# joshspeagle/frankenz

Measured on AMD Instinct MI355X. Metric: object-template likelihood evals/sec (fused fit_predict -> PDFs), higher is better.
Workload: dtype f64 throughout (chi2, ln-likes, every weight, ln-evidence, PDFs; an fp32 estimate of the weight only CLASSIFIES which pairs can matter to an fp64 sum, DESIGN.md 3.1)

## Files before the change

### frankenz_amd/csrc/fz_hist.h

```cpp
#pragma once
#include <type_traits>
#include "fz_kernels.h"
#include "fz_nolist.h"

namespace fz {

#define FZ_HEXP_K 256
#ifndef FZ_HIST_MP
#define FZ_HIST_MP 1
#endif
#ifndef FZ_HIST_TILE384
#define FZ_HIST_TILE384 1
#endif
#ifndef FZ_HIST_REFRESH_TILE
#define FZ_HIST_REFRESH_TILE 1
#endif
#ifndef FZ_HIST_STAGE_LATE
#define FZ_HIST_STAGE_LATE 1
#endif
#ifndef FZ_HIST_SETTLE2
#define FZ_HIST_SETTLE2 0
#endif
#ifndef FZ_HIST_SEG_NW0
#define FZ_HIST_SEG_NW0 16
#endif
#ifndef FZ_HIST_SEG_PFMAX
#define FZ_HIST_SEG_PFMAX 12
#endif
#ifndef FZ_HIST_REFRESH
#define FZ_HIST_REFRESH 32
#endif
#ifndef FZ_HIST_LEAN
#define FZ_HIST_LEAN 1
#endif
#ifndef FZ_HIST_AHEAD
#define FZ_HIST_AHEAD 1
#endif
#ifndef FZ_HIST_WAIT_EARLY
#define FZ_HIST_WAIT_EARLY 0
#endif
#ifndef FZ_HIST_SEAM
#define FZ_HIST_SEAM 1
#endif
#ifndef FZ_HIST_PRIO
#define FZ_HIST_PRIO 1
#endif
constexpr int hist_prio_level(int policy, int pos) {
    return policy == 1 ? (pos < 2 ? 3 : (pos < 4 ? 2 : (pos < 5 ? 1 : 0)))
         : policy == 2 ? (pos < 3 ? 1 : 0)
         : policy == 3 ? (pos < 2 ? 1 : 0)
         : 0;
}
#ifndef FZ_HIST_PRIO_FORMS
#define FZ_HIST_PRIO_FORMS (2 | 4 | 8 | 16)
#endif
constexpr int hist_prio_step(int pos, int ns) { return ns < 2 ? 0 : (3 * (ns - 1 - pos) + ns - 2) / (ns - 1); }
__device__ __forceinline__ void hist_setprio(int p) {
    switch (p) {
        case 0: __builtin_amdgcn_s_setprio(0); break;
        case 1: __builtin_amdgcn_s_setprio(1); break;
        case 2: __builtin_amdgcn_s_setprio(2); break;
        default: __builtin_amdgcn_s_setprio(3); break;
    }
}
#ifdef FZ_HIST_WSTATS
static __device__ unsigned long long fz_hwstats[16 * 12];
#define FZ_HIST_WSTATS_ON 1
inline void hist_wstats_print(hipStream_t stream, int nb, long long n, long long M, long long blocks, int nw) {
    unsigned long long h[16 * 12], z[16 * 12] = {0};
    (void)hipStreamSynchronize(stream);
    (void)hipMemcpyFromSymbol(h, HIP_SYMBOL(fz_hwstats), sizeof h);
    (void)hipMemcpyToSymbol(HIP_SYMBOL(fz_hwstats), z, sizeof z);
    fprintf(stderr, "HWSTATS k_hist<%d bands>: n %lld M %lld, %lld blocks x %d waves\n", nb, n, M, blocks, nw);
    for (int r = 0; r < nw / 4; ++r) {
        double s[5] = {0, 0, 0, 0, 0};
        char simd[128]; int q = 0;
        for (int w = 4 * r; w < 4 * r + 4; ++w) {
            const unsigned long long* e = h + w * 12;
            for (int k = 0; k < 5; ++k) s[k] += (double)e[k];
            q += snprintf(simd + q, sizeof simd - q, " w%d:%llu/%llu/%llu/%llu", w, e[8], e[9], e[10], e[11]);
        }
        const double life = s[4] > 0 ? s[4] : 1.0;
        fprintf(stderr, "HWSTATS rank %d (waves %d-%d): life %.4g cycles per wave | tile barrier %.2f %% | round barriers %.2f %% | finish %.2f %% | "
                        "prologue %.2f %% | per wave, tile barrier %%:", r, 4 * r, 4 * r + 3, s[4] / (4.0 * (double)(h[4 * r * 12 + 5] ? h[4 * r * 12 + 5] : 1)),
                100 * s[0] / life, 100 * s[1] / life, 100 * s[2] / life, 100 * s[3] / life);
        for (int w = 4 * r; w < 4 * r + 4; ++w) fprintf(stderr, " %.2f", 100.0 * (double)h[w * 12] / (double)(h[w * 12 + 4] ? h[w * 12 + 4] : 1));
        fprintf(stderr, " | launches on SIMD 0/1/2/3:%s\n", simd);
    }
}
#else
#define FZ_HIST_WSTATS_ON 0
#endif
template <bool L>
__device__ __forceinline__ double fma3(double a, double b, double c) {
    if constexpr (L) { double d; asm("v_fma_f64 %0, %1, %2, %3" : "=v"(d) : "v"(a), "v"(b), "v"(c)); return d; }
    else return fma(a, b, c);
}
template <bool L>
__device__ __forceinline__ double fma3_sb(double a, double b, double c) {
    if constexpr (L) { double d; asm("v_fma_f64 %0, %1, %2, %3" : "=v"(d) : "v"(a), "s"(b), "v"(c)); return d; }
    else return fma(a, b, c);
}
template <bool L>
__device__ __forceinline__ double fma3_mhalf(double a, double c) {
    if constexpr (L) { double d; asm("v_fma_f64 %0, %1, -0.5, %2" : "=v"(d) : "v"(a), "v"(c)); return d; }
    else return fma(a, -0.5, c);
}
template <bool L>
__device__ __forceinline__ int exp_insert(int hi, int n) {
    if constexpr (L) { int r; asm("v_lshl_add_u32 %0, %1, 12, %2" : "=v"(r) : "v"(n & ~(FZ_HEXP_K - 1)), "v"(hi)); return r; }
    else return hi + ((n >> 8) << 20);
}
struct ExpK {
    double c1 = 369.3299304675746;
    double c2 = -0.0027076061740622863;
    double c6 = 1.0 / 6.0;
};
template <bool NEGONLY = false, bool L = false>
__device__ __forceinline__ double exp_small_tab(double x, const double* __restrict__ tab, const ExpK& ek = ExpK()) {
    const double MAGIC = 6755399441055744.0;
    x = NEGONLY ? vmax_raw(x, -700.0) : vmin_raw(vmax_raw(x, -700.0), 700.0);
    const double d = fma(x, ek.c1, MAGIC);
    const double r = fma(d - MAGIC, ek.c2, x);
    const int n = __double2loint(d);
    const double t = tab[n & (FZ_HEXP_K - 1)];
    double p = fma3_sb<L>(r, 1.0 / 120.0, 1.0 / 24.0);
    p = fma3<L>(p, r, ek.c6);
    p = fma(p, r, 0.5);
    p = fma(p, r, 1.0);
    p = fma(p, r, 1.0);
    const double v = t * p;
    static_assert(FZ_HEXP_K == 256, "the exponent insert shifts n by log2 of the table's length");
    return __hiloint2double(exp_insert<L>(__double2hiint(v), n), __double2loint(v));
}

__device__ __forceinline__ double sqrt_nr(double r) {
    const double y = __builtin_amdgcn_rsq(vmax_raw(r, 1e-300));
    const double hy = 0.5 * y;
    double s = r * y;
    s = fma(fma(-s, s, r), hy, s);
    s = fma(fma(-s, s, r), hy, s);
    return s;
}
constexpr double hist_ln(double k) {
    return k == 1.0 ? 0.0 : k == 2.0 ? 0.6931471805599453 : k == 3.0 ? 1.0986122886681098 : k == 4.0 ? 1.3862943611198906
         : k == 5.0 ? 1.6094379124341003 : k == 6.0 ? 1.791759469228055 : k == 7.0 ? 1.9459101090932196 : 2.0794415416798357;
}
template <int WP, bool SMALL = false, bool L = false>
__device__ __forceinline__ double hist_exactw(double c2, const FastTabs& tb, const ExpK& ek = ExpK()) {
    constexpr double K = (double)WP;
    const double r = c2 * (1.0 / K);
    double pw = 1.0;
    if constexpr ((WP >> 1) <= 3) {
        if constexpr ((WP >> 1) >= 1) pw = r;
        if constexpr ((WP >> 1) >= 2) pw = pw * r;
        if constexpr ((WP >> 1) >= 3) pw = pw * r;
    } else {
        double base = r;
#pragma unroll
        for (int e = WP >> 1; e > 0; e >>= 1) { if (e & 1) pw = pw * base; base = base * base; }
    }
    if constexpr (SMALL && (WP >> 1) <= 3) {
        double q = 1.0;
        if constexpr ((WP >> 1) >= 1) q = c2;
        if constexpr ((WP >> 1) >= 2) q = q * c2;
        if constexpr ((WP >> 1) >= 3) q = q * c2;
        if constexpr (WP & 1) {
            const double y = __builtin_amdgcn_rsq(c2), hy = 0.5 * y;
            double sq = c2 * y;
            sq = fma(fma(-sq, sq, c2), hy, sq);
            sq = fma(fma(-sq, sq, c2), hy, sq);
            q = (WP >> 1) ? q * sq : sq;
        }
        constexpr double EK = 0.5 * K - 0.5 * K * hist_ln(K);
        return q * exp_small_tab<true, L>(fma3_mhalf<L>(c2, EK), tb.expt, ek);
    }
    if constexpr (!SMALL && (WP >> 1) <= 3) {
        double q = 1.0;
        if constexpr ((WP >> 1) >= 1) q = c2;
        if constexpr ((WP >> 1) >= 2) q = q * c2;
        if constexpr ((WP >> 1) >= 3) q = q * c2;
        if constexpr (WP & 1) q = (WP >> 1) ? q * sqrt_nr(c2) : sqrt_nr(c2);
        constexpr double EK = 0.5 * K - 0.5 * K * hist_ln(K);
        return q * exp_neg(fma(c2, -0.5, EK), tb);
    }
    if constexpr (WP & 1) pw = pw * sqrt_nr(r);
    const double w = pw * (SMALL ? exp_small_tab(fma(c2, -0.5, 0.5 * K), tb.expt) : exp_clamped(fma(c2, -0.5, 0.5 * K), tb));
    if constexpr ((WP >> 1) > 3) return (c2 < K + 1400.0) ? w : 0.0;
    else return w;
}

template <bool SMALL = false>
__device__ __forceinline__ double hist_exactw_rt(double c2, int wp, const FastTabs& tb) {
    const double K = (double)wp;
    if (wp == 0) return SMALL ? exp_small_tab(-0.5 * c2, tb.expt) : exp_clamped(-0.5 * c2, tb);
    const double r = c2 * rcp_nr<2>(K);
    double pw = 1.0, base = r;
    for (int e = wp >> 1; e > 0; e >>= 1) { if (e & 1) pw = pw * base; base = base * base; }
    if (wp & 1) pw = pw * sqrt_nr(r);
    const double w = pw * (SMALL ? exp_small_tab(fma(c2, -0.5, 0.5 * K), tb.expt) : exp_clamped(fma(c2, -0.5, 0.5 * K), tb));
    return (c2 < K + 1400.0) ? w : 0.0;
}

template <bool SMALL = false>
__device__ __forceinline__ double hist_exactw_rt8(double c2, int wp, double K, double rK, const FastTabs& tb) {
    if (wp == 0) return SMALL ? exp_small_tab<true>(-0.5 * c2, tb.expt) : exp_clamped(-0.5 * c2, tb);
    const double r = c2 * rK, r2 = r * r;
    const int h = wp >> 1;
    double pw = ((h & 1) ? r : 1.0) * ((h & 2) ? r2 : 1.0);
    if (wp & 1) pw = pw * sqrt_nr(r);
    return pw * (SMALL ? exp_small_tab<true>(fma(c2, -0.5, 0.5 * K), tb.expt) : exp_clamped(fma(c2, -0.5, 0.5 * K), tb));
}

template <class SRC>
constexpr int hist_tile() {
    if (FZ_HIST_SETTLE2 && SRC::NB <= 8 && SRC::RW <= 6 && SRC::LMODE == 1) return 128;
    if (FZ_HIST_TILE384 && SRC::NB <= 8 && SRC::RW <= 6) return 384;
    if (SRC::NB <= 8) return (SRC::RW <= 10 && !(SRC::LMODE == 2 && SRC::RW > 6)) ? 256 : 128;
    return SRC::RW <= 18 ? 256 : (SRC::RW <= 34 ? 128 : 64);
}
template <class SRC>
constexpr bool hist_prefetch() {
    if (SRC::NB <= 8) return SRC::NB + SRC::NVAL <= 18;
    return 2 * SRC::NB + 2 * SRC::RW <= 96;
}

__device__ __forceinline__ float wave_maxf_dpp(float v) {
    int x = __float_as_int(v);
    auto mx = [](int a, int b) { float r; asm("v_max_f32 %0, %1, %2" : "=v"(r) : "v"(__int_as_float(a)), "v"(__int_as_float(b))); return __float_as_int(r); };
    x = mx(x, __builtin_amdgcn_update_dpp(x, x, 0xB1, 0xf, 0xf, false));
    x = mx(x, __builtin_amdgcn_update_dpp(x, x, 0x4E, 0xf, 0xf, false));
    x = mx(x, __builtin_amdgcn_update_dpp(x, x, 0x141, 0xf, 0xf, false));
    x = mx(x, __builtin_amdgcn_update_dpp(x, x, 0x140, 0xf, 0xf, false));
    const float a = __int_as_float(__builtin_amdgcn_readlane(x, 0)), b = __int_as_float(__builtin_amdgcn_readlane(x, 16));
    const float c = __int_as_float(__builtin_amdgcn_readlane(x, 32)), d = __int_as_float(__builtin_amdgcn_readlane(x, 48));
    return fmaxf(fmaxf(a, b), fmaxf(c, d));
}

__device__ __forceinline__ double wave_max_pos_hi(double v) {
    int x = __double2hiint(v);
    auto mx = [](int a, int b) { return a > b ? a : b; };
    x = mx(x, __builtin_amdgcn_update_dpp(x, x, 0xB1, 0xf, 0xf, false));
    x = mx(x, __builtin_amdgcn_update_dpp(x, x, 0x4E, 0xf, 0xf, false));
    x = mx(x, __builtin_amdgcn_update_dpp(x, x, 0x141, 0xf, 0xf, false));
    x = mx(x, __builtin_amdgcn_update_dpp(x, x, 0x140, 0xf, 0xf, false));
    const int a = __builtin_amdgcn_readlane(x, 0), b = __builtin_amdgcn_readlane(x, 16), c = __builtin_amdgcn_readlane(x, 32), d = __builtin_amdgcn_readlane(x, 48);
    return __hiloint2double(mx(mx(a, b), mx(c, d)), 0);
}

#ifndef FZ_HIST_CHI2_2OP
#define FZ_HIST_CHI2_2OP 1
#endif
#ifndef FZ_HIST_C2ZERO
#define FZ_HIST_C2ZERO 1e-16
#endif

template <int TW>
struct HistState {
    double S[TW];
    double Sc[TW];
    double wmx[TW];
    float tmax[TW];
    float tthr[TW];
    double wamb[TW];
    int pend[TW];
    int namb[TW];
    int tick, next;
};

template <class SRC>
struct HistArgs {
    SRC src;
    KdeView kv;
    int64_t N;
    double* lmap; double* levid; double* pdfs;
    const int* omap; int* redo; const int* order;
    int normalize;
};
template <class SRC, int TW, int NW, bool EXACT, bool OBJK = (SRC::NB > 8), bool SEG = false>
__global__ __launch_bounds__(NW * 64) void k_hist(HistArgs<SRC> a_, const KdeView* __restrict__ kvp, int acc_stride, int M,
                                                   double wt_thresh, Cand* __restrict__ amb, int64_t cap) {
    constexpr bool LEAN = (FZ_HIST_LEAN == 1) && !SEG;
    constexpr bool AHD = (FZ_HIST_AHEAD == 1) && LEAN && !EXACT && !(FZ_HIST_SETTLE2 == 1) && !OBJK && SRC::RW <= 6;
    constexpr bool WE = (FZ_HIST_WAIT_EARLY == 1) && AHD;
    constexpr bool SEAM = (FZ_HIST_SEAM == 1) && AHD && hist_prefetch<SRC>() && (FZ_HIST_STAGE_LATE == 1);
    auto hq = [&]() -> const HistArgs<SRC>& {
        if constexpr (!LEAN) return a_;
        auto p = __builtin_amdgcn_kernarg_segment_ptr();
        asm volatile("" : "+s"(p));
        return *(const HistArgs<SRC>*)p;
    };
    const int64_t N = a_.N;
    constexpr int TILE = hist_tile<SRC>(), RW = SRC::RW, TDR = RW * TILE, TD = TDR + TILE / 2, NT = NW * 64, OD = SRC::OBJ_DOUBLES;
    constexpr int WP = SRC::WPOW, BT = SRC::NB;
    constexpr int PRIO = (SEAM && TILE == 384 && (BT == 5 || (FZ_HIST_PRIO_FORMS & 16))) ? FZ_HIST_PRIO : 0;
    constexpr int PFORM = SEG ? 8 : (OBJK ? 2 : (EXACT ? 4 : 1));
    constexpr bool PWORSE = (SEG && !EXACT && SRC::LMODE == 0 && BT == 4) || (OBJK && !SEG && !EXACT && BT == 8);
    constexpr bool PRIOF = (FZ_HIST_PRIO > 0) && !SEAM && BT <= 8 && (FZ_HIST_PRIO_FORMS & PFORM) != 0 && !PWORSE;
    constexpr bool WST = (FZ_HIST_WSTATS_ON == 1) && SEAM;
    [[maybe_unused]] unsigned long long wst_a = 0, wst_b = 0, wst_c = 0, wst_d = 0;
    auto wclk = [&]() -> unsigned long long { if constexpr (WST) return __builtin_readcyclecounter(); else return 0ull; };
    [[maybe_unused]] const unsigned long long wst_life = wclk();
    static_assert(!OBJK || TW == 1, "per-object band counts: one object per wave");
    static_assert(!SEG || (OBJK && SRC::NB <= 8), "segments: run-time band counts, 4-8 bands");
    constexpr double SEG_VBIG = BT <= 5 ? 0x1p192 : (BT == 6 ? 0x1p160 : (BT == 7 ? 0x1p137 : 0x1p120));
    constexpr int KOFF = SRC::LMODE == 2 ? 3 : 2;
    constexpr bool KRT = OBJK;
    int wpr = WP;
    double K = (double)WP;
    bool kok = true;
    double lgq = a_.src.lp.lg_full;
    constexpr int NOBJ = NW * TW;
    constexpr bool S2 = (FZ_HIST_SETTLE2 == 1) && !EXACT && SRC::NB <= 8 && SRC::RW <= 6 && SRC::LMODE == 1;
    constexpr int CAP = S2 ? 192 : 128, DTHR = CAP - 64;
    using tag_t = uint16_t;
    static_assert(WP >= 1 && WP <= 30, "chi2^(1/2) ... chi2^15");
    __shared__ __attribute__((aligned(16))) double tileA[TD];
    __shared__ __attribute__((aligned(16))) double tileB[TD];
    __shared__ __attribute__((aligned(16))) double s_c2[EXACT ? 2 : NOBJ * CAP];
    __shared__ tag_t s_tag[EXACT ? 2 : NOBJ * CAP];
    __shared__ __attribute__((aligned(16))) double s_tabs[EXACT ? FZ_TABS_DOUBLES : FZ_HEXP_K];
    __shared__ __attribute__((aligned(16))) double s_objs[EXACT ? NOBJ * OD : 2];
    __shared__ __attribute__((aligned(16))) double s_obj0[SEG ? NOBJ * OD : 2];
    static_assert(EXACT || TW * OD <= TW * CAP, "an object row must fit its candidate buffer");
    extern __shared__ double s_rows[];
    const int tid = threadIdx.x, lane = tid & 63;
    const int wave = __builtin_amdgcn_readfirstlane(tid >> 6);
    const int64_t nwaves = (int64_t)gridDim.x * NW, gw = (int64_t)blockIdx.x * NW + wave;
    const int64_t ngroups = (N + TW - 1) / TW, nrounds = (ngroups + nwaves - 1) / nwaves;
    const int ntiles = (M + TILE - 1) / TILE;
    SRC src = a_.src;
    src.tb = global_tabs();
    const FastTabs tb = src.tb;
    FastTabs tbx;
    if constexpr (EXACT) tbx = stage_tabs(s_tabs, tid, NT);
    else {
        for (int k = tid; k < FZ_HEXP_K; k += NT) s_tabs[k] = FZ_EXP_TAB[k * (FZ_EXP_K / FZ_HEXP_K)];
        tbx.logt = nullptr; tbx.expt = s_tabs;
    }
    const KdeView kv = [&]() { if constexpr (SEG) return *kvp; else return a_.kv; }();
    const int32_t* posw = SEG ? kv.mc_tag : kv.pos;
    const int w0 = SEG ? 0 : kv.w0;
    double* objs = EXACT ? s_objs + wave * (TW * OD) : s_c2 + wave * (TW * CAP);
    double* obj0 = s_obj0 + (SEG ? wave * (TW * OD) : 0);
    double* rows = s_rows + (size_t)wave * TW * acc_stride;
    double* rc2 = s_c2 + (EXACT ? 0 : wave * (TW * CAP));
    tag_t* rtag = s_tag + (EXACT ? 0 : wave * (TW * CAP));
    Cand* ambw = amb + (size_t)gw * TW * cap;
    auto t_consts = [](double Kd, float& hk23, float& T0c, float& tmarg) {
        const double hk = 0.5 * Kd;
        hk23 = (float)(hk / 8388608.0);
        T0c = (float)((Kd > 0.0 ? -hk * log2(Kd) : 0.0) + Kd * 0.7213475204444817 + hk * (-127.0 + 0.043));
        tmarg = (float)(0.5 + 0.045 * hk);
    };
    float hk23, T0c, tmarg;
    t_consts(K, hk23, T0c, tmarg);
    float tzero = K > 0.0 ? -INFINITY : T0c;
    const float lthr2 = (wt_thresh > 0.0) ? (float)log2(wt_thresh) : -INFINITY;
    int mbits = 0;
    while (((int64_t)1 << mbits) < (int64_t)M) ++mbits;
    const float ldrop0 = fminf(lthr2, -(float)(55 + mbits));
    const double thr_def = wt_thresh * (1.0 + 1e-3);
    auto lnl_c2 = [&](double c2) {
        if constexpr (KRT) return (wpr == 0) ? fma(-0.5, c2, -lgq) : chi2_logpdf<true>(0.5 * K, c2, lgq, tb);
        else return src.lnl_of_chi2(c2);
    };
    double rK = 1.0;
    ExpK ek;
    if constexpr (LEAN) asm volatile("" : "+s"(ek.c1), "+s"(ek.c2), "+v"(ek.c6));
    auto exactw_tab = [&](double c2, const FastTabs& t, auto small) {
        if constexpr (SEG) {
            if constexpr (SRC::LMODE == 2) { if (wpr == WP) return hist_exactw<WP, decltype(small)::value>(c2, t); }
            return hist_exactw_rt8<decltype(small)::value>(c2, wpr, K, rK, t);
        }
        else if constexpr (KRT) return hist_exactw_rt<decltype(small)::value>(c2, wpr, t);
        else return hist_exactw<WP, decltype(small)::value, LEAN>(c2, t, ek);
    };
    double lref = uniform_d(lnl_c2(K));
    auto obj_of = [&](const HistArgs<SRC>& h, int64_t s) -> int64_t {
        if constexpr (!EXACT && !SEG) {
            if (h.order) { const int64_t q = (int64_t)h.order[s]; s = q < 0 ? 0 : (q < h.N ? q : h.N - 1); }
        }
        return h.omap ? (int64_t)h.omap[s] : s;
    };

    for (int64_t rnd = 0; rnd < nrounds; ++rnd) {
        const int64_t g = gw + rnd * nwaves;
        const bool work = g < ngroups;
        [[maybe_unused]] const unsigned long long wst_r0 = wclk();
        const int64_t i0 = work ? g * TW : 0;
        const HistArgs<SRC>& hp = hq();
        [[maybe_unused]] const SRC& srcp = hp.src;
#pragma unroll
        for (int o = 0; o < TW; ++o) {
            const int64_t os = i0 + o < hp.N ? i0 + o : hp.N - 1;
            srcp.park_obj(obj_of(hp, os), objs + o * OD, lane);
        }
        for (int k = lane; k < TW * acc_stride; k += 64) rows[k] = 0.0;
        uint32_t obits = 0; double oslv = 0.0, fk = 1.0; int segcur = -1, ndcur = 0;
        bool segbad = false;
        int nbadm = 0;
        auto seg_lnl = [&](double c2, int nd) {
            const bool dp = src.lp.dim_prior != 0;
            const int wp = dp ? nd - KOFF : 0;
            const double lg = dp ? src.lp.lgtab[nd] : 0.5 * ((double)nd * FZ_LN2PI + oslv);
            const double xl = (wp == 0) ? 0.0 : (0.5 * (double)wp) * log_pos_t<true>(c2, tb);
            return fma(-0.5, c2, xl) - lg;
        };
        if constexpr (SEG) {
            const int64_t os = i0 < hp.N ? i0 : hp.N - 1;
            const int64_t oi = obj_of(hp, os);
            src.park_obj(oi, obj0, lane);
            if constexpr ((SRC::LMODE == 1 || SRC::LMODE == 2) && FZ_HIST_CHI2_2OP && !(SRC::LMODE == 2 && SRC::SAFE)) {
                if (lane < BT) { const double sv = sqrt(obj0[BT + lane]); obj0[BT + lane] = sv; obj0[lane] = obj0[lane] * sv; }
            }
            obits = (uint32_t)__builtin_amdgcn_readfirstlane((int)src.ov.bits[oi]);
            oslv = uniform_d(src.ov.slv[oi]);
            const bool dp = src.lp.dim_prior != 0;
            double lr = -INFINITY; bool bad = false;
            for (int sg = lane; sg < kv.seg_n; sg += 64) {
                const int nd = __popc(obits & kv.seg_mask[sg]);
                const int wp = dp ? nd - KOFF : 0;
                bad |= wp < -1;
                nbadm += (wp == -1) ? kv.seg_start[sg + 1] - kv.seg_start[sg] : 0;
                const double lg = dp ? src.lp.lgtab[nd] : 0.5 * ((double)nd * FZ_LN2PI + oslv);
                const double hw = 0.5 * (double)wp;
                if (wp >= 0) lr = fmax(lr, wp > 0 ? fma(hw, log_pos((double)wp, tb), -hw) - lg : -lg);
            }
            nbadm = __builtin_amdgcn_readfirstlane((int)wave_sum((double)nbadm));
            kok = __ballot(bad) == 0ull && nbadm <= (M >> 3);
            lref = uniform_d(wave_max(lr));
            float h_, t_; t_consts((double)BT, h_, t_, tmarg);
            tmarg = uniform_f(tmarg);
        }
        if constexpr (OBJK && !SEG) {
            const int64_t os = i0 < hp.N ? i0 : hp.N - 1;
            const int64_t oi = obj_of(hp, os);
            const int nb = __builtin_amdgcn_readfirstlane(__popc(srcp.ov.bits[oi]));
            wpr = nb - (SRC::LMODE == 2 ? 3 : 2);
            kok = wpr >= 0;
            if (!kok) wpr = 1;
            const bool dp = src.lp.dim_prior != 0;
            if (!dp) { wpr = 0; kok = true; }
            K = uniform_d((double)wpr);
            t_consts(K, hk23, T0c, tmarg);
            hk23 = uniform_f(hk23); T0c = uniform_f(T0c); tmarg = uniform_f(tmarg);
            tzero = wpr > 0 ? -INFINITY : T0c;
            lgq = uniform_d(dp ? srcp.lp.lgtab[nb] : 0.5 * ((double)nb * FZ_LN2PI + srcp.ov.slv[oi]));
            lref = uniform_d(lnl_c2(K));
        }
        int tid0 = tid;
        if constexpr (SEAM) asm volatile("" : "+v"(tid0));
        nl_stage_tile<SRC, TILE, NT, true>(src, posw, 0, tileA, tid0, wave);
        if constexpr (WST) {
            const unsigned long long t1 = wclk();
// ... 333 lines not shown
                    if constexpr (SLOW) { const int lim = flush ? 1 : DTHR; while (hs.pend[o] >= lim) drain(o, std::true_type{}, lane); }
                    else { while (hs.pend[o] >= DTHR) drain(o, std::false_type{}, lane); }
#endif
                        }
                    }
                }
        };
        auto tile_barrier = [&]() {
#if !defined(FZ_DIAG_NOBARRIER)
            if constexpr (WST) {
                const unsigned long long t0 = wclk();
                __syncthreads();
                wst_a += wclk() - t0;
            } else
            __syncthreads();
#endif
        };
        [[maybe_unused]] typename SRC::MR mseam[MP];
        [[maybe_unused]] int tagseam[MP];
        auto run_tile = [&](const double* cur, double* nxt, int t, auto tailc, auto slowc) {
            constexpr bool TAIL = decltype(tailc)::value;
            constexpr bool pure = !decltype(slowc)::value;
            constexpr bool LATE = FZ_HIST_STAGE_LATE && pure && hist_prefetch<SRC>() && !(SEG && SRC::NB + SRC::NVAL > FZ_HIST_SEG_PFMAX);
            if (!LATE || !work) { if (t + 1 < ntiles) nl_stage_tile<SRC, TILE, NT, true>(src, posw, t + 1, nxt, tid, wave); }
            if (work) {
                const int32_t* tags = reinterpret_cast<const int32_t*>(cur + TDR);
                static_assert((TILE / 64) % MP == 0, "groups per trip must divide the tile");
                constexpr bool PF = hist_prefetch<SRC>() && !(SEG && SRC::NB + SRC::NVAL > FZ_HIST_SEG_PFMAX);
                if constexpr (pure) {
                    typename SRC::MR mn[PF ? MP : 1];
                    int tagn[MP];
                    if constexpr (SEAM) {
#pragma unroll
                        for (int q = 0; q < MP; ++q) { mn[q] = mseam[q]; tagn[q] = tagseam[q]; }
                    } else if constexpr (PF) {
#pragma unroll
                        for (int q = 0; q < MP; ++q) {
                            src.template load_model_lds<TILE>(cur, q * 64 + lane, mn[q]);
                            tagn[q] = tags[q * 64 + lane];
                        }
                    }
                    if constexpr (LATE) { if (t + 1 < ntiles) nl_stage_tile<SRC, TILE, NT, true>(src, posw, t + 1, nxt, tid, wave); }
#pragma unroll
                    for (int st = 0; st < TILE / 64; st += MP) {
                        typename SRC::MR m[MP];
                        int ptag[MP];
#pragma unroll
                        for (int q = 0; q < MP; ++q) {
                            if constexpr (PF) { m[q] = mn[q]; ptag[q] = tagn[q]; }
                            else { src.template load_model_lds<TILE>(cur, (st + q) * 64 + lane, m[q]); ptag[q] = tags[(st + q) * 64 + lane]; }
                            asm volatile("" : "+v"(ptag[q]));
                        }
                        if (PF && st + MP < TILE / 64) {
#pragma unroll
                            for (int q = 0; q < MP; ++q) {
                                src.template load_model_lds<TILE>(cur, (st + MP + q) * 64 + lane, mn[q]);
                                tagn[q] = tags[(st + MP + q) * 64 + lane];
                            }
                        }
                        if constexpr (SEAM) {
                            if (st + MP >= TILE / 64) {
                                tile_barrier();
                                if constexpr (!TAIL) {
                                    const int32_t* tagx = reinterpret_cast<const int32_t*>(nxt + TDR);
#pragma unroll
                                    for (int q = 0; q < MP; ++q) {
                                        src.template load_model_lds<TILE>(nxt, q * 64 + lane, mseam[q]);
                                        tagseam[q] = tagx[q * 64 + lane];
                                    }
                                }
                            }
                        }
                        if constexpr (PRIO >= 1 && PRIO <= 3) hist_setprio(hist_prio_level(PRIO, st + MP >= TILE / 64 ? 0 : st + 1));
                        if constexpr (PRIO == 5) { if (st == 0) hist_setprio(((wave >> 2) + t) & 3); }
                        if constexpr (PRIOF) hist_setprio(hist_prio_step(st / MP, TILE / 64 / MP));
                        if constexpr (AHD && PF) __builtin_amdgcn_sched_barrier(0);
                        step_body(m, ptag, st, t, tailc, std::false_type{}, false);
                    }
                } else {
                    {
#pragma unroll 1
                        for (int st = -1; st < TILE / 64; ++st) {
                            typename SRC::MR m[MP];
                            int ptag[MP];
                            const int stc = st < 0 ? 0 : st;
                            src.template load_model_lds<TILE>(cur, stc * 64 + lane, m[0]);
                            ptag[0] = st < 0 ? (int)0x80000000 : tags[stc * 64 + lane];
                            const int nxt = st + 1 < TILE / 64 ? (tags[(st + 1) * 64] >> 16) & 0x3fff : segcur;
                            if (st >= 0) {
                                const int sw = (__builtin_amdgcn_readfirstlane(ptag[0]) >> 16) & 0x7fff;
                                if ((sw & 0x3fff) != segcur) {
                                    if (mcw && segcur >= 0) {
                                        const int rko = kv.seg_rank[segcur];
                                        if (kv.seg_rank[sw & 0x3fff] != rko) { const HistArgs<SRC>& hc = hq(); class_flush(rko, rows, hc.pdfs + obj_of(hc, i0) * kv.G); }
                                    }
                                    seg_switch(sw);
                                }
                            }
                            const bool flush = __builtin_amdgcn_readfirstlane(nxt) != segcur;
                            step_body(m, ptag, stc, t, tailc, std::true_type{}, flush);
                        }
                    }
                }
                if constexpr (FZ_HIST_REFRESH_TILE && !EXACT) {
                    if (++hs.tick == hs.next) { hs.next = hs.tick < 3 ? hs.tick + 1 : hs.tick + 5; refresh_bars(); }
                }
            }
            if constexpr (SEAM && pure) { if (!work) tile_barrier(); }
            else tile_barrier();
        };
        if constexpr (SEAM) {
            if (work) {
                const int32_t* tag0 = reinterpret_cast<const int32_t*>(tileA + TDR);
#pragma unroll
                for (int q = 0; q < MP; ++q) {
                    src.template load_model_lds<TILE>(tileA, q * 64 + lane, mseam[q]);
                    tagseam[q] = tag0[q * 64 + lane];
                }
            }
        }
        if constexpr (PRIO == 4) { if (work) hist_setprio(wave >> 2); }
        if constexpr (!SEG) {
            for (int t = 0; t < ntiles; t += 2) {
                if (t + 1 < ntiles) run_tile(tileA, tileB, t, std::false_type{}, std::false_type{}); else run_tile(tileA, tileB, t, std::true_type{}, std::false_type{});
                if (t + 1 < ntiles) {
                    if (t + 2 < ntiles) run_tile(tileB, tileA, t + 1, std::false_type{}, std::false_type{}); else run_tile(tileB, tileA, t + 1, std::true_type{}, std::false_type{});
                }
            }
        } else {
            auto tile_pure = [&](const double* cur) -> bool {
                if (!work) return true;
                const int wv = (reinterpret_cast<const int32_t*>(cur + TDR)[(lane % (TILE / 64)) * 64] >> 16) & 0x7fff;
                return __ballot(wv != segcur) == 0ull && !segbad;
            };
            int t = 0;
            while (t < ntiles) {
                if (!(t & 1)) {
                    while (t < ntiles) {
                        if (!tile_pure(tileA)) break;
                        run_tile(tileA, tileB, t, std::false_type{}, std::false_type{}); ++t;
                        if (t >= ntiles || !tile_pure(tileB)) break;
                        run_tile(tileB, tileA, t, std::false_type{}, std::false_type{}); ++t;
                    }
                    if (t >= ntiles) break;
                }
                if (t & 1) run_tile(tileB, tileA, t, std::false_type{}, std::true_type{});
                else run_tile(tileA, tileB, t, std::false_type{}, std::true_type{});
                ++t;
            }
        }

        if constexpr (PRIO > 0 || PRIOF) __builtin_amdgcn_s_setprio(0);
        [[maybe_unused]] const unsigned long long wst_f0 = wclk();
        if (work) {
#pragma unroll 1
            for (int o = 0; o < TW; ++o) {
                const HistArgs<SRC>& hf = hq();
                const KdeView& kvf = SEG ? kv : hf.kv;
                if (i0 + o >= hf.N) break;
                const int64_t i = obj_of(hf, i0 + o);
                double* const pdfs = hf.pdfs;
                auto lnl_fin = [&](double c2) {
                    if constexpr (KRT || !LEAN) return lnl_c2(c2);
                    else return chi2_logpdf<true>(0.5 * WP, c2, hf.src.lp.lg_full, tb);
                };
                double lrf = lref;
                if constexpr (!KRT && LEAN) lrf = uniform_d(lnl_fin(K));
                double* row = rows + o * acc_stride;
                double wbest_run = 0.0;
                int lanef = lane;
                if constexpr (SEAM) asm volatile("" : "+v"(lanef));
                if constexpr (!EXACT) {
                    while (hs.pend[o] > 0) drain(o, std::integral_constant<bool, SEG>{}, lanef);
                } else {
                    wbest_run = wave_max(hs.Sc[o]);
                }
                if constexpr (!EXACT) wbest_run = wave_max(hs.wmx[o]);
                const double lbest = (wbest_run > 0.0) ? uniform_d(lrf + log_pos(wbest_run, tb)) : -INFINITY;
                const double stot = wave_sum(EXACT ? hs.S[o] : hs.Sc[o]);
                const double le = lrf + log_pos(stot, tb);
                const float tm = EXACT ? 0.f : wave_maxf(hs.tmax[o]);
                const bool ok = (le - le == 0.0) && (lbest > -INFINITY) && (EXACT ? (wbest_run > 1e-24) : (tm >= -400.f)) && hs.namb[o] >= 0 && kok;
                if constexpr (SEG) { if (mcw && segcur >= 0) class_flush(kv.seg_rank[segcur], row, pdfs + i * kv.G); }
                const int na = __builtin_amdgcn_readfirstlane(hs.namb[o]);
                if (na > 0) {
                    __builtin_amdgcn_fence(__ATOMIC_RELEASE, "workgroup");
                    __builtin_amdgcn_fence(__ATOMIC_ACQUIRE, "agent");
                    const double thr = wt_thresh * exp_neg(lbest - le, tb);
                    const Cand* cb = ambw + (size_t)o * cap;
                    for (int c0 = 0; c0 < na; c0 += 64) {
                        const int k = c0 + lane;
                        const bool in1 = k < na;
                        const Cand e1 = cb[in1 ? k : 0];
                        double l1, w1;
                        if constexpr (SEG) {
                            l1 = in1 ? seg_lnl(e1.lnl, e1.pad & 0xff) : -INFINITY;
                            w1 = exp_neg(l1 - lref, tb);
                        } else {
                            l1 = in1 ? lnl_fin(e1.lnl) : -INFINITY;
                            w1 = exactw_tab(e1.lnl, tb, std::false_type{});
                        }
                        const bool s1 = in1 && (exp_neg(l1 - le, tb) > thr);
                        if constexpr (SEG) {
                            if (mcw) {
                                if (s1) {
                                    const int rk = e1.pad >> 8, wc = kv.mc_width[rk], p = e1.j - kv.mc_w0;
                                    const double* kr = kv.kern + kv.mc_off[rk];
                                    const double wn = w1 * kv.mc_norm[(size_t)rk * kv.mc_gp + e1.j];
                                    const int G = (int)kv.G;
                                    for (int h = 0; h <= 2 * wc; ++h) {
                                        const int tq = p - wc + h;
                                        if (tq >= 0 && tq < G) unsafeAtomicAdd(&row[tq], wn * kr[h]);
                                    }
                                }
                                continue;
                            }
                        }
                        if (s1) unsafeAtomicAdd(&row[e1.j + w0], w1);
                    }
                }
                if (lane == 0) {
                    if (hf.lmap) hf.lmap[i] = lbest;
                    if (hf.levid) hf.levid[i] = le;
                    if (!ok) hf.redo[1 + atomicAdd(hf.redo, 1)] = (int)i;
                }
                if constexpr (SEG) {
                    if (mcw) {
                        double* gout = pdfs + i * kv.G;
                        const int G = (int)kv.G;
                        if (!ok) { for (int tq = lane; tq < G; tq += 64) gout[tq] = NAN; continue; }
                        double tot = 0.0;
                        for (int tq = lane; tq < G; tq += 64) { const double vq = gout[tq] + row[tq]; row[tq] = vq; tot += vq; }
                        tot = wave_sum(tot);
                        const int normalize = hf.normalize;
                        const double sc = normalize ? 1.0 / tot : 1.0 / stot;
                        for (int tq = lane; tq < G; tq += 64) gout[tq] = normalize ? row[tq] / tot : row[tq] * sc;
                        continue;
                    }
                }
                kde_finalize<true>(kvf, row, ok, hf.normalize, pdfs + i * kvf.G, lanef, ok ? 1.0 / stot : 1.0, true);
            }
        }
        if constexpr (WST) {
            const unsigned long long t1 = wclk();
            __syncthreads();
            wst_c += t1 - wst_f0; wst_b += wclk() - t1;
        } else
        __syncthreads();
    }
    if constexpr (WST) {
#ifdef FZ_HIST_WSTATS
        const unsigned long long life = wclk() - wst_life;
        const int simd = (int)__builtin_amdgcn_s_getreg((1 << 11) | (4 << 6) | 4);
        if (lane == 0 && wave < 16) {
            unsigned long long* h = fz_hwstats + wave * 12;
            atomicAdd(h + 0, wst_a); atomicAdd(h + 1, wst_b); atomicAdd(h + 2, wst_c); atomicAdd(h + 3, wst_d);
            atomicAdd(h + 4, life); atomicAdd(h + 5, 1ull); atomicAdd(h + 6, (unsigned long long)nrounds);
            atomicAdd(h + 8 + (simd & 3), 1ull);
        }
#endif
    }
}

}
```

### frankenz_amd/csrc/fz_kernels.h

```cpp
#pragma once
#include "fz_device.h"

namespace fz {

struct PlaneSrc {
    const double* p; int64_t ld;
    FastTabs tb;
    static constexpr int WPOW = 0;
    struct MR {};
    struct OR { const double* row; };
    __device__ __forceinline__ void load_model(int64_t, MR&) const {}
    __device__ __forceinline__ void load_obj(int64_t i, OR& o) const { o.row = p + i * ld; }
    __device__ __forceinline__ void load_obj_fresh(int64_t i, OR& o) const { o.row = p + i * ld; }
    __device__ __forceinline__ double lnl(const OR& o, const MR&, int64_t j, bool valid) const {
        return valid ? o.row[j] : -INFINITY;
    }
};
template <int BT, int MODE, int VAR, int PRI = 0>
struct PhotSrc : Phot<BT, MODE, VAR> {
    using P = Phot<BT, MODE, VAR>;
    static constexpr int WPOW = (VAR == VAR_FAST && !PRI) ? (MODE == 2 ? BT - 3 : BT - 2) : 0;
    static constexpr bool HAS_PRIOR = PRI != 0;
    static constexpr int NB = BT;
    static constexpr int LMODE = MODE;
// ... 128 lines not shown
                if (MPT == 1) {
                    if (lnl) __builtin_nontemporal_store(r[u][0].lnl, &lnl[k]);
                    if (chi2) __builtin_nontemporal_store(r[u][0].chi2, &chi2[k]);
                    if (ndim) __builtin_nontemporal_store((int64_t)r[u][0].ndim, &ndim[k]);
                    if (scale) __builtin_nontemporal_store(r[u][0].scale, &scale[k]);
                    if (serr) __builtin_nontemporal_store(sqrt(1.0 / r[u][0].shape), &serr[k]);
                } else {
                    const PairOut &a = r[u][0], &b = r[u][MPT - 1];
                    if (lnl) __builtin_nontemporal_store(fz_d2{a.lnl, b.lnl}, reinterpret_cast<fz_d2*>(&lnl[k]));
                    if (chi2) __builtin_nontemporal_store(fz_d2{a.chi2, b.chi2}, reinterpret_cast<fz_d2*>(&chi2[k]));
                    if (ndim) __builtin_nontemporal_store(fz_l2{a.ndim, b.ndim}, reinterpret_cast<fz_l2*>(&ndim[k]));
                    if (scale) __builtin_nontemporal_store(fz_d2{a.scale, b.scale}, reinterpret_cast<fz_d2*>(&scale[k]));
                    if (serr) __builtin_nontemporal_store(fz_d2{sqrt(1.0 / a.shape), sqrt(1.0 / b.shape)},
                                                          reinterpret_cast<fz_d2*>(&serr[k]));
                }
            }
        }
    }
}

typedef double fz_d2l __attribute__((ext_vector_type(2)));
struct KdeView {
    int64_t G;
    int kmode;
    const int32_t* pos;
    const int32_t* cls;
    const double* norm;
    const double* normtab;
    const int64_t* widths; const int64_t* offsets; const double* kern;
    int32_t w0; int64_t koff0;
    const double* ly; const double* lstd; const int32_t* lo; const int32_t* hi;
    const double* grid;
    double gstep;
    const double* lrec;
    int acc_stride;
    int lane_window;
    const int32_t* mc_tag; const int32_t* mc_width; const int64_t* mc_off; const double* mc_norm;
    int32_t mc_gp, mc_w0;
    const uint32_t* seg_mask; const int32_t* seg_rank; const int32_t* seg_start; int32_t seg_n, seg_nrank;
};
enum { KDE_HIST = 0, KDE_DICT = 1, KDE_GRID = 2 };

#define FZ_LANE_WINDOW 160
__device__ __forceinline__ void kde_scatter(const KdeView& kv, double* row, bool sel, double w, int64_t jm,
                                            int lane) {
    if (kv.kmode == KDE_HIST) {
        if (sel) unsafeAtomicAdd(&row[kv.pos[jm] + kv.w0], w / kv.norm[jm]);
        return;
    }
    bool wide = false;
    if (kv.kmode == KDE_DICT) {
        if (sel) {
            const int p = kv.pos[jm], c = kv.cls[jm];
            const int wd = (int)kv.widths[c];
            const int lo = max(p - wd, 0), hi = min(p + wd + 1, (int)kv.G);
            wide = hi - lo > kv.lane_window;
            if (!wide) {
                const double wn = w / kv.norm[jm];
                const double* kr = kv.kern + kv.offsets[c] + (lo - (p - wd)) - lo;
                for (int t = lo; t < hi; ++t) unsafeAtomicAdd(&row[t], wn * kr[t]);
            }
        }
    } else if (kv.gstep > 0.0) {
        if (sel) {
            const fz_d2l* rec = reinterpret_cast<const fz_d2l*>(kv.lrec + 6 * jm);
            const fz_d2l ra = rec[0], rb = rec[1], rc = rec[2];
            const int lo = __double2loint(rc.x), hi = __double2hiint(rc.x);
            wide = hi - lo > kv.lane_window;
            if (!wide && rb.x != 0.0) {
                const double mu = ra.x, isd = ra.y, q = rb.y;
                const double wg = w * rb.x, h = kv.gstep * isd;
                const FastTabs tb = global_tabs();
                for (int t0 = lo; t0 < hi; t0 += 64) {
                    const double z = (kv.grid[t0] - mu) * isd;
                    double g = wg * exp_neg(-0.5 * (z * z), tb);
                    double r = exp_clamped(-fma(z, h, 0.5 * (h * h)), tb);
                    const int t1 = min(t0 + 64, hi);
                    for (int t = t0; t < t1; ++t) { unsafeAtomicAdd(&row[t], g); g *= r; r *= q; }
                }
            }
        }
    } else {
        if (sel) {
            const int lo = kv.lo[jm], hi = kv.hi[jm];
            const double nrm = kv.norm[jm];
            wide = hi - lo > kv.lane_window;
            if (!wide && nrm != 0.0) {
                const double mu = kv.ly[jm], sd = kv.lstd[jm];
                const double isd = 1.0 / sd;
                const double wg = (w / nrm) / (2.5066282746310002 * sd);
                for (int t = lo; t < hi; ++t) {
                    const double z = (kv.grid[t] - mu) * isd;
                    unsafeAtomicAdd(&row[t], wg * exp_neg(-0.5 * (z * z)));
                }
            }
        }
    }
    int lo = 0, hi = 0, kidx = 0;
    double pa = 0.0, pb = 0.0;
    double pc = 0.0;
    if (wide) {
        if (kv.kmode == KDE_DICT) {
            const int p = kv.pos[jm], c = kv.cls[jm];
            const int wd = (int)kv.widths[c];
            lo = max(p - wd, 0); hi = min(p + wd + 1, (int)kv.G);
            kidx = (int)kv.offsets[c] + (lo - (p - wd)) - lo;
            pa = w / kv.norm[jm];
        } else {
            const double nrm = kv.norm[jm], sd = kv.lstd[jm];
            lo = kv.lo[jm]; hi = (nrm != 0.0) ? kv.hi[jm] : lo;
            pa = (w / nrm) / (2.5066282746310002 * sd);
            pb = 1.0 / sd;
            pc = kv.ly[jm];
        }
    }
    auto rl = [](double v, int l) {
        return __hiloint2double(__builtin_amdgcn_readlane(__double2hiint(v), l), __builtin_amdgcn_readlane(__double2loint(v), l));
    };
    unsigned long long mask = __ballot(wide);
    constexpr int UM = 4;
    while (mask) {
        int lo_u[UM], hi_u[UM], k_u[UM]; double a_u[UM], b_u[UM], c_u[UM], v_u[UM];
#pragma unroll
        for (int u = 0; u < UM; ++u) {
            if (mask) {
                const int sl = __builtin_ctzll(mask);
                mask &= mask - 1;
                lo_u[u] = __builtin_amdgcn_readlane(lo, sl); hi_u[u] = __builtin_amdgcn_readlane(hi, sl);
                k_u[u] = __builtin_amdgcn_readlane(kidx, sl);
                a_u[u] = rl(pa, sl); b_u[u] = rl(pb, sl); c_u[u] = rl(pc, sl);
            } else { lo_u[u] = 0; hi_u[u] = 0; k_u[u] = 0; a_u[u] = b_u[u] = c_u[u] = 0.0; }
        }
#pragma unroll
        for (int u = 0; u < UM; ++u) {
            const int t = lo_u[u] + lane;
            v_u[u] = 0.0;
            if (t < hi_u[u]) v_u[u] = (kv.kmode == KDE_DICT) ? kv.kern[k_u[u] + t] : kv.grid[t];
        }
#pragma unroll
        for (int u = 0; u < UM; ++u) {
            const int t = lo_u[u] + lane;
            if (t < hi_u[u]) {
                if (kv.kmode == KDE_DICT) row[t] += a_u[u] * v_u[u];
                else { const double z = (v_u[u] - c_u[u]) * b_u[u]; row[t] += a_u[u] * exp_neg(-0.5 * (z * z)); }
            }
            for (int t2 = t + 64; t2 < hi_u[u]; t2 += 64) {
                if (kv.kmode == KDE_DICT) row[t2] += a_u[u] * kv.kern[k_u[u] + t2];
                else { const double z = (kv.grid[t2] - c_u[u]) * b_u[u]; row[t2] += a_u[u] * exp_neg(-0.5 * (z * z)); }
            }
        }
    }
}

template <bool HO = false>
__device__ __forceinline__ void kde_finalize(const KdeView& kv, double* row, bool ok, int normalize,
                                             double* out, int lane, double scale = 1.0, bool bymass = false) {
    const int G = (int)kv.G;
    if (!ok) { for (int t = lane; t < G; t += 64) out[t] = NAN; return; }
    double tot = 0.0;
    if (HO || kv.kmode == KDE_HIST) {
        const int w2 = 2 * kv.w0;
        if (bymass) { for (int k = lane; k < G + w2; k += 64) row[k] = row[k] / kv.normtab[k]; }
        const double* kr = kv.kern + kv.koff0;
        if (w2 < 128) {
            const double ka = (lane <= w2) ? kr[lane] : 0.0;
            const double kb = (lane + 64 <= w2) ? kr[lane + 64] : 0.0;
            const int kal = __double2loint(ka), kah = __double2hiint(ka), kbl = __double2loint(kb), kbh = __double2hiint(kb);
            for (int t = lane; t < G; t += 128) {
                const bool two = t + 64 < G;
                const double* r0 = row + t;
                const double* r1 = row + (two ? t + 64 : t);
                double v0 = 0.0, v1 = 0.0;
                const int hs = w2 < 64 ? 0 : w2 - 63;
                for (int h = 0; h < hs; ++h) {
                    const int q = w2 - h - 64;
                    const double tap = __hiloint2double(__builtin_amdgcn_readlane(kbh, q), __builtin_amdgcn_readlane(kbl, q));
                    v0 = fma(r0[h], tap, v0); v1 = fma(r1[h], tap, v1);
                }
                for (int h = hs; h <= w2; ++h) {
                    const int q = w2 - h;
                    const double tap = __hiloint2double(__builtin_amdgcn_readlane(kah, q), __builtin_amdgcn_readlane(kal, q));
                    v0 = fma(r0[h], tap, v0); v1 = fma(r1[h], tap, v1);
                }
                tot += v0;
                if (two) tot += v1;
                if (normalize) { row[t] = v0; if (two) row[t + 64] = v1; }
                else { out[t] = v0 * scale; if (two) out[t + 64] = v1 * scale; }
            }
        } else {
            for (int t = lane; t < G; t += 64) {
                double v = 0.0;
                for (int h = 0; h <= w2; ++h) v = fma(row[t + h], kr[w2 - h], v);
                out[t] = normalize ? v : v * scale;
                tot += v;
            }
            if (normalize) {
                tot = wave_sum(tot);
                for (int t = lane; t < G; t += 64) out[t] = out[t] / tot;
            }
            return;
        }
    } else {
        for (int t = lane; t < G; t += 64) { const double v = row[t]; tot += v; if (!normalize) out[t] = v * scale; }
    }
    if (normalize) {
        tot = wave_sum(tot);
        for (int t = lane; t < G; t += 64) out[t] = row[t] / tot;
    }
}

template <class SRC, int TW>
__global__ __launch_bounds__(256) void k_stats(SRC src_, int64_t N, int64_t M, int linear,
                                               double* __restrict__ lmap, double* __restrict__ levid) {
    SRC src = src_;
    src.tb = global_tabs();
    const int wave = __builtin_amdgcn_readfirstlane(threadIdx.x >> 6);
    const int lane = threadIdx.x & 63;
    const int64_t i0 = ((int64_t)blockIdx.x * (blockDim.x >> 6) + wave) * TW;
    if (i0 >= N) return;
    typename SRC::OR ob[TW];
    MS st[TW];
    unsigned firstnan = 0, anynan = 0;
#pragma unroll
    for (int o = 0; o < TW; ++o) {
        src.load_obj(i0 + o < N ? i0 + o : N - 1, ob[o]);
        ms_init(st[o]);
    }
    for (int64_t jb = 0; jb < M; jb += 64) {
        const int64_t j = jb + lane;
        const bool valid = j < M;
        typename SRC::MR m;
        src.load_model(j, m);
#pragma unroll
        for (int o = 0; o < TW; ++o) {
            const double l = src.lnl(ob[o], m, j, valid);
            if (l != l) { anynan |= 1u << o; if (j == 0) firstnan |= 1u << o; }
            if (linear) { if (l > st[o].m) st[o].m = l; }
            else ms_push(st[o], l, src.tb);
        }
    }
#pragma unroll
    for (int o = 0; o < TW; ++o) {
        const int64_t i = i0 + o;
        const bool fn = __any((firstnan >> o) & 1u);
        const bool an = __any((anynan >> o) & 1u);
        if (linear) {
            const double mx = wave_max(st[o].m);
            if (lane == 0 && i < N) lmap[i] = an ? (double)NAN : mx;
        } else {
            MS t = wave_ms(st[o]);
            if (lane == 0 && i < N) {
                lmap[i] = fn ? (double)NAN : t.m;
                if (levid) levid[i] = an ? (double)NAN : (t.m == INFINITY ? (double)INFINITY : t.m + log(t.s));
            }
        }
    }
}

template <class SRC, int TW>
__global__ __launch_bounds__(256) void k_kde(SRC src_, KdeView kv, int64_t N, int64_t M, int linear,
                                             const double* __restrict__ lmap,
                                             const double* __restrict__ levid, double wt_thresh,
                                             int normalize, double* __restrict__ pdfs) {
    extern __shared__ double smem[];
    SRC src = src_;
    src.tb = global_tabs();
    const int wave = __builtin_amdgcn_readfirstlane(threadIdx.x >> 6);
    const int lane = threadIdx.x & 63;
    const int64_t i0 = ((int64_t)blockIdx.x * (blockDim.x >> 6) + wave) * TW;
    if (i0 >= N) return;
    double* acc = smem + (size_t)wave * TW * kv.acc_stride;
    for (int k = lane; k < TW * kv.acc_stride; k += 64) acc[k] = 0.0;

    typename SRC::OR ob[TW];
    double le[TW], thr[TW], lthr[TW];
    bool ok[TW];
#pragma unroll
    for (int o = 0; o < TW; ++o) {
        const int64_t i = i0 + o < N ? i0 + o : N - 1;
        src.load_obj(i, ob[o]);
        const double lm = lmap[i];
        if (linear) {
            le[o] = 0.0;
            ok[o] = (i0 + o < N);
            thr[o] = wt_thresh * lm;
            lthr[o] = -INFINITY;
        } else {
            le[o] = levid[i];
            ok[o] = (i0 + o < N) && (le[o] - le[o] == 0.0);
            thr[o] = wt_thresh * exp_neg(lm - le[o], src.tb);
            lthr[o] = (wt_thresh > 0.0) ? lm + log(wt_thresh) - 1e-3 : -INFINITY;
        }
    }
    for (int64_t jb = 0; jb < M; jb += 64) {
        const int64_t j = jb + lane;
        const bool valid = j < M;
        typename SRC::MR m;
        src.load_model(j, m);
#pragma unroll
        for (int o = 0; o < TW; ++o) {
            if (!ok[o]) continue;
            const double l = src.lnl(ob[o], m, j, valid);
            const bool cand = valid && (linear ? true : (l >= lthr[o]));
            if (!__any(cand)) continue;
            const double w = linear ? l : exp_neg(l - le[o], src.tb);
            const bool sel = cand && (w > thr[o]);
            kde_scatter(kv, acc + o * kv.acc_stride, sel, w, j, lane);
        }
    }
#pragma unroll
    for (int o = 0; o < TW; ++o) {
        const int64_t i = i0 + o;
        if (i >= N) break;
        kde_finalize(kv, acc + o * kv.acc_stride, ok[o], normalize, pdfs + i * kv.G, lane);
    }
}

typedef __attribute__((address_space(3))) void lds_void;
typedef __attribute__((address_space(1))) const void gbl_cvoid;

struct Cand { double lnl; int32_t j; int32_t pad; };
#define FZ_RES 4


template <int TW>
struct FusedState {
    MS st[TW];
    int cnt[TW];
    unsigned firstnan, anynan;
    int tick;
};

template <class SRC, int TW, int DPT, bool TAIL, int TL>
__device__ __forceinline__ void fused_tile(const SRC& src, const FastTabs& tb, const double* cur, const double* objs,
                                           int jt0, int M, int lane, double lt, Cand* buf, int64_t cap,
                                           FusedState<TW>& fs) {
    constexpr int OD = SRC::OBJ_DOUBLES;
#pragma unroll 1
    for (int s = 0; s < TL / 64; ++s) {
        const int j = jt0 + s * 64 + lane;
        typename SRC::MR m;
        src.template load_model_lds<TL>(cur, s * 64 + lane, m);
        double l[TW];
#pragma unroll
        for (int o = 0; o < TW; ++o) {
            typename SRC::OR ob;
            src.load_obj_lds(objs + o * OD, ob);
            l[o] = src.template lnl_t<DPT>(ob, m, j, TAIL ? (j < M) : true);
            if (TAIL) l[o] = (j < M) ? l[o] : -INFINITY;
        }
#pragma unroll
        for (int o = 0; o < TW; ++o) {
            if constexpr (!SRC::NO_NAN) {
                if (l[o] != l[o]) { fs.anynan |= 1u << o; if (j == 0) fs.firstnan |= 1u << o; }
            }
            ms_push(fs.st[o], l[o], tb);
        }
#pragma unroll
        for (int o = 0; o < TW; ++o) {
            bool c = l[o] >= fs.st[o].m + lt;
// ... 644 lines not shown
```

Baseline: 726.0 billion.

## Add register-blocked histogram finish row with sliding-window convolution

Adds a specialised per-row finish path (hist_finish_row) for the histogram kernel in the 1-mode, no-segment, up-to-5-band case. It batches the normtab division with unrolled loads, then runs the kernel-smoothing convolution with each lane owning a contiguous block of 12 outputs. A sliding register window replaces re-reading row memory for every tap. The normalisation sums and writes come from registers, and the wave-stats instrumentation gains finish-phase checkpoints. The cost is higher register pressure and a fallback to the old path for wide kernels or large grids.

```diff
diff --git a/frankenz_amd/csrc/fz_hist.h b/frankenz_amd/csrc/fz_hist.h
--- a/frankenz_amd/csrc/fz_hist.h
+++ b/frankenz_amd/csrc/fz_hist.h
@@ -41,6 +41,9 @@
 #endif
 #ifndef FZ_HIST_SEAM
 #define FZ_HIST_SEAM 1
+#endif
+#ifndef FZ_HIST_FINISH
+#define FZ_HIST_FINISH 1
 #endif
 #ifndef FZ_HIST_PRIO
 #define FZ_HIST_PRIO 1
@@ -64,28 +67,31 @@
     }
 }
 #ifdef FZ_HIST_WSTATS
-static __device__ unsigned long long fz_hwstats[16 * 12];
+static __device__ unsigned long long fz_hwstats[16 * 16];
 #define FZ_HIST_WSTATS_ON 1
 inline void hist_wstats_print(hipStream_t stream, int nb, long long n, long long M, long long blocks, int nw) {
-    unsigned long long h[16 * 12], z[16 * 12] = {0};
+    unsigned long long h[16 * 16], z[16 * 16] = {0};
     (void)hipStreamSynchronize(stream);
     (void)hipMemcpyFromSymbol(h, HIP_SYMBOL(fz_hwstats), sizeof h);
     (void)hipMemcpyToSymbol(HIP_SYMBOL(fz_hwstats), z, sizeof z);
     fprintf(stderr, "HWSTATS k_hist<%d bands>: n %lld M %lld, %lld blocks x %d waves\n", nb, n, M, blocks, nw);
     for (int r = 0; r < nw / 4; ++r) {
-        double s[5] = {0, 0, 0, 0, 0};
+        double s[5] = {0, 0, 0, 0, 0}, c[4] = {0, 0, 0, 0};
         char simd[128]; int q = 0;
         for (int w = 4 * r; w < 4 * r + 4; ++w) {
-            const unsigned long long* e = h + w * 12;
+            const unsigned long long* e = h + w * 16;
             for (int k = 0; k < 5; ++k) s[k] += (double)e[k];
+            for (int k = 0; k < 4; ++k) c[k] += (double)e[12 + k];
             q += snprintf(simd + q, sizeof simd - q, " w%d:%llu/%llu/%llu/%llu", w, e[8], e[9], e[10], e[11]);
         }
         const double life = s[4] > 0 ? s[4] : 1.0;
         fprintf(stderr, "HWSTATS rank %d (waves %d-%d): life %.4g cycles per wave | tile barrier %.2f %% | round barriers %.2f %% | finish %.2f %% | "
-                        "prologue %.2f %% | per wave, tile barrier %%:", r, 4 * r, 4 * r + 3, s[4] / (4.0 * (double)(h[4 * r * 12 + 5] ? h[4 * r * 12 + 5] : 1)),
+                        "prologue %.2f %% | per wave, tile barrier %%:", r, 4 * r, 4 * r + 3, s[4] / (4.0 * (double)(h[4 * r * 16 + 5] ? h[4 * r * 16 + 5] : 1)),
                 100 * s[0] / life, 100 * s[1] / life, 100 * s[2] / life, 100 * s[3] / life);
-        for (int w = 4 * r; w < 4 * r + 4; ++w) fprintf(stderr, " %.2f", 100.0 * (double)h[w * 12] / (double)(h[w * 12 + 4] ? h[w * 12 + 4] : 1));
+        for (int w = 4 * r; w < 4 * r + 4; ++w) fprintf(stderr, " %.2f", 100.0 * (double)h[w * 16] / (double)(h[w * 16 + 4] ? h[w * 16 + 4] : 1));
         fprintf(stderr, " | launches on SIMD 0/1/2/3:%s\n", simd);
+        fprintf(stderr, "HWSTATS rank %d finish: c1 %.2f %% | c2 %.2f %% | c3 %.2f %% | c4 %.2f %% of the waves' life\n", r,
+                100 * c[0] / life, 100 * c[1] / life, 100 * c[2] / life, 100 * c[3] / life);
     }
 }
 #else
@@ -301,6 +307,11 @@
     [[maybe_unused]] unsigned long long wst_a = 0, wst_b = 0, wst_c = 0, wst_d = 0;
     auto wclk = [&]() -> unsigned long long { if constexpr (WST) return __builtin_readcyclecounter(); else return 0ull; };
     [[maybe_unused]] const unsigned long long wst_life = wclk();
+    [[maybe_unused]] unsigned long long wst_cp[4] = {0, 0, 0, 0}, wst_last = 0;
+    [[maybe_unused]] auto wmark = [&](int k) {
+        if constexpr (WST) { const unsigned long long now = wclk(); wst_cp[k - 1] += now - wst_last; wst_last = now; }
+    };
+    constexpr bool FIN = (FZ_HIST_FINISH == 1) && !SEG && !OBJK && SRC::LMODE == 1 && SRC::NB <= 5;
     static_assert(!OBJK || TW == 1, "per-object band counts: one object per wave");
     static_assert(!SEG || (OBJK && SRC::NB <= 8), "segments: run-time band counts, 4-8 bands");
     constexpr double SEG_VBIG = BT <= 5 ? 0x1p192 : (BT == 6 ? 0x1p160 : (BT == 7 ? 0x1p137 : 0x1p120));
@@ -940,6 +951,7 @@
 
         if constexpr (PRIO > 0 || PRIOF) __builtin_amdgcn_s_setprio(0);
         [[maybe_unused]] const unsigned long long wst_f0 = wclk();
+        if constexpr (WST) wst_last = wst_f0;
         if (work) {
 #pragma unroll 1
             for (int o = 0; o < TW; ++o) {
@@ -1026,7 +1038,12 @@
                         continue;
                     }
                 }
-                kde_finalize<true>(kvf, row, ok, hf.normalize, pdfs + i * kvf.G, lanef, ok ? 1.0 / stot : 1.0, true);
+                if constexpr (WST) {
+                    if constexpr (FIN) hist_finish_row<12>(kvf, row, ok, hf.normalize, pdfs + i * kvf.G, lanef, ok ? 1.0 / stot : 1.0, wmark);
+                    else kde_finalize<true>(kvf, row, ok, hf.normalize, pdfs + i * kvf.G, lanef, ok ? 1.0 / stot : 1.0, true, wmark);
+                    wmark(4);
+                } else if constexpr (FIN) hist_finish_row<12>(kvf, row, ok, hf.normalize, pdfs + i * kvf.G, lanef, ok ? 1.0 / stot : 1.0);
+                else kde_finalize<true>(kvf, row, ok, hf.normalize, pdfs + i * kvf.G, lanef, ok ? 1.0 / stot : 1.0, true);
             }
         }
         if constexpr (WST) {
@@ -1041,10 +1058,11 @@
         const unsigned long long life = wclk() - wst_life;
         const int simd = (int)__builtin_amdgcn_s_getreg((1 << 11) | (4 << 6) | 4);
         if (lane == 0 && wave < 16) {
-            unsigned long long* h = fz_hwstats + wave * 12;
+            unsigned long long* h = fz_hwstats + wave * 16;
             atomicAdd(h + 0, wst_a); atomicAdd(h + 1, wst_b); atomicAdd(h + 2, wst_c); atomicAdd(h + 3, wst_d);
             atomicAdd(h + 4, life); atomicAdd(h + 5, 1ull); atomicAdd(h + 6, (unsigned long long)nrounds);
             atomicAdd(h + 8 + (simd & 3), 1ull);
+            for (int k = 0; k < 4; ++k) atomicAdd(h + 12 + k, wst_cp[k]);
         }
 #endif
     }
diff --git a/frankenz_amd/csrc/fz_kernels.h b/frankenz_amd/csrc/fz_kernels.h
--- a/frankenz_amd/csrc/fz_kernels.h
+++ b/frankenz_amd/csrc/fz_kernels.h
@@ -304,15 +304,18 @@
     }
 }
 
-template <bool HO = false>
+struct NoMark { __device__ __forceinline__ void operator()(int) const {} };
+template <bool HO = false, class MK = NoMark>
 __device__ __forceinline__ void kde_finalize(const KdeView& kv, double* row, bool ok, int normalize,
-                                             double* out, int lane, double scale = 1.0, bool bymass = false) {
+                                             double* out, int lane, double scale = 1.0, bool bymass = false, MK mk = MK{}) {
     const int G = (int)kv.G;
     if (!ok) { for (int t = lane; t < G; t += 64) out[t] = NAN; return; }
     double tot = 0.0;
     if (HO || kv.kmode == KDE_HIST) {
         const int w2 = 2 * kv.w0;
+        mk(1);
         if (bymass) { for (int k = lane; k < G + w2; k += 64) row[k] = row[k] / kv.normtab[k]; }
+        mk(2);
         const double* kr = kv.kern + kv.koff0;
         if (w2 < 128) {
             const double ka = (lane <= w2) ? kr[lane] : 0.0;
@@ -339,6 +342,7 @@
                 if (normalize) { row[t] = v0; if (two) row[t + 64] = v1; }
                 else { out[t] = v0 * scale; if (two) out[t + 64] = v1 * scale; }
             }
+            mk(3);
         } else {
             for (int t = lane; t < G; t += 64) {
                 double v = 0.0;
@@ -346,6 +350,7 @@
                 out[t] = normalize ? v : v * scale;
                 tot += v;
             }
+            mk(3);
             if (normalize) {
                 tot = wave_sum(tot);
                 for (int t = lane; t < G; t += 64) out[t] = out[t] / tot;
@@ -358,6 +363,116 @@
     if (normalize) {
         tot = wave_sum(tot);
         for (int t = lane; t < G; t += 64) out[t] = row[t] / tot;
+    }
+}
+
+template <int NACC = 12, class MK = NoMark, int QB = 2>
+__device__ __forceinline__ void hist_finish_row(const KdeView& kv, double* row, bool ok, int normalize, double* out, int lane,
+                                                double scale, MK mk = MK{}) {
+    const int G = (int)kv.G, w2 = 2 * kv.w0;
+    if (w2 >= 128 || G > 64 * NACC) { kde_finalize<true>(kv, row, ok, normalize, out, lane, scale, true, mk); return; }
+    if (!ok) { for (int t = lane; t < G; t += 64) out[t] = NAN; return; }
+    constexpr int UG = 4;
+    constexpr int NQ = (64 * NACC + 126 + 63) / 64;
+    constexpr int NQG = (NQ + UG - 1) / UG;
+    const int n = G + w2, last = n - 1;
+    mk(1);
+#pragma unroll
+    for (int b = 0; b < NQG; b += QB) {
+        double rv[QB * UG], nv[QB * UG];
+#pragma unroll
+        for (int g = 0; g < QB; ++g) {
+            if (64 * UG * (b + g) < n) {
+#pragma unroll
+                for (int u = 0; u < UG; ++u) {
+                    const int k = min(lane + 64 * (UG * (b + g) + u), last);
+                    nv[UG * g + u] = kv.normtab[k]; rv[UG * g + u] = row[k];
+                }
+            }
+        }
+#pragma unroll
+        for (int g = 0; g < QB; ++g) {
+            if (64 * UG * (b + g) < n) {
+#pragma unroll
+                for (int u = 0; u < UG; ++u) {
+                    const int k = lane + 64 * (UG * (b + g) + u);
+                    const double q = rv[UG * g + u] / nv[UG * g + u];
+                    if (k < n) row[k] = q;
+                }
+            }
+        }
+    }
+    mk(2);
+    __builtin_amdgcn_wave_barrier();
+    const double* kr = kv.kern + kv.koff0;
+    const double ka = (lane <= w2) ? kr[lane] : 0.0;
+    const double kb = (lane + 64 <= w2) ? kr[lane + 64] : 0.0;
+    const int kal = __double2loint(ka), kah = __double2hiint(ka), kbl = __double2loint(kb), kbh = __double2hiint(kb);
+    const int base = NACC * min(lane, (G - 1) / NACC);
+    const int room = last - base;
+    const double* r0 = row + base;
+    double acc[NACC], win[NACC];
+#pragma unroll
+    for (int a = 0; a < NACC; ++a) { acc[a] = 0.0; win[a] = r0[min(a, room)]; }
+    for (int h = 0; h <= w2; h += NACC) {
+#pragma unroll
+        for (int u = 0; u < NACC; ++u) {
+            if (h + u <= w2) {
+                const int q = w2 - (h + u);
+                const double tap = (q < 64) ? __hiloint2double(__builtin_amdgcn_readlane(kah, q), __builtin_amdgcn_readlane(kal, q))
+                                            : __hiloint2double(__builtin_amdgcn_readlane(kbh, q - 64), __builtin_amdgcn_readlane(kbl, q - 64));
+#pragma unroll
+                for (int a = 0; a < NACC; ++a) acc[a] = fma(win[(a + u) % NACC], tap, acc[a]);
+                win[u] = r0[min(NACC + h + u, room)];
+            }
+        }
+    }
+    __builtin_amdgcn_wave_barrier();
+#pragma unroll
+    for (int a = 0; a < NACC; ++a) { if (NACC * lane + a < G) row[NACC * lane + a] = acc[a]; }
+    __builtin_amdgcn_wave_barrier();
+    constexpr int NOG = (NACC + UG - 1) / UG;
+    double val[NOG * UG];
+    double tot = 0.0;
+#pragma unroll
+    for (int g = 0; g < NOG; ++g) {
+        if (64 * UG * g < G) {
+#pragma unroll
+            for (int u = 0; u < UG; ++u) val[UG * g + u] = row[min(lane + 64 * (UG * g + u), G - 1)];
+        }
+    }
+#pragma unroll
+    for (int g = 0; g < NOG; ++g) {
+        if (64 * UG * g < G) {
+#pragma unroll
+            for (int u = 0; u < UG; ++u) { if (lane + 64 * (UG * g + u) < G) tot += val[UG * g + u]; }
+        }
+    }
+    mk(3);
+    if (normalize) {
+        tot = wave_sum(tot);
+#pragma unroll
+        for (int g = 0; g < NOG; ++g) {
+            if (64 * UG * g < G) {
+#pragma unroll
+                for (int u = 0; u < UG; ++u) {
+                    const int t = lane + 64 * (UG * g + u);
+                    const double v = val[UG * g + u] / tot;
+                    if (t < G) out[t] = v;
+                }
+            }
+        }
+    } else {
+#pragma unroll
+        for (int g = 0; g < NOG; ++g) {
+            if (64 * UG * g < G) {
+#pragma unroll
+                for (int u = 0; u < UG; ++u) {
+                    const int t = lane + 64 * (UG * g + u);
+                    if (t < G) out[t] = val[UG * g + u] * scale;
+                }
+            }
+        }
     }
 }
 
```

New measurement: 754.0 billion, median of 6. +3.9%, better.
